# koide3/glim

Measured on NVIDIA H100. Metric: VGICP linearize throughput, higher is better.
Workload: dtype f32

## Files before the change

glim_b200/csrc/gb_api.cu:

```cuda
#include "gb_internal.cuh"
#include "gb_grid_math.cuh"

#include <stdarg.h>
#include <stdio.h>
#include <stdlib.h>
#include <string.h>

#include <algorithm>
#include <atomic>
#include <cmath>
#include <map>
#include <mutex>
#include <new>
#include <thread>

static thread_local char g_err[512] = "";
void gb_set_error(const char* fmt, ...) {
  va_list ap;
  va_start(ap, fmt);
  vsnprintf(g_err, sizeof(g_err), fmt, ap);
  va_end(ap);
}
extern "C" const char* gb_last_error(void) { return g_err; }
extern "C" const char* gb_status_string(gb_status s) {
// ... 327 lines not shown
  return GB_OK;
}

static gb_status grid_factor_args(const gb_ctx* ctx, const gb_point_grid* target, const gb_cloud* source, double max_correspondence_distance, bool icp, gb_factor** out,
                                  float* max_corr2, int* half_width) {
  GB_REQUIRE(ctx && target && source && out, "null argument");
  *out = nullptr;
  GB_REQUIRE(std::isfinite(max_correspondence_distance) && max_correspondence_distance > 0.0, "max_correspondence_distance must be positive and finite");
  const gb_voxelmap* m = grid_map(target);
  GB_REQUIRE(m->kind == GB_MAP_POINTS, "the target is not a point grid (gb_point_grid_build)");
  GB_REQUIRE(m->device == ctx->device && source->device == ctx->device, "cloud / point grid live on another device");
  GB_REQUIRE(icp || source->covs, "the source carries no covariances");
  *max_corr2 = (float)(max_correspondence_distance * max_correspondence_distance);
  *half_width = grid_half_width(m->inv_res, *max_corr2, m->key_extent);
  GB_REQUIRE(*half_width <= kGridMaxHalfWidth, "max_correspondence_distance / cell_size too large: the search would span more than 17^3 cells");
  return GB_OK;
}
extern "C" gb_status gb_gicp_grid_factor_create(gb_ctx* ctx, const gb_point_grid* target, const gb_cloud* source, double max_correspondence_distance, gb_factor** out) {
  float max_corr2 = 0.f;
  int half_width = 0;
  GB_CHECK(grid_factor_args(ctx, target, source, max_correspondence_distance, false, out, &max_corr2, &half_width));
  GB_ENTER(ctx);
  gb_factor* f = factor_new(ctx, GB_FACTOR_POSE, grid_map(target), source);
  if (!f) return GB_ERR_INTERNAL;
  f->max_corr2 = max_corr2;
  f->grid_m = half_width;
  *out = f;
  return GB_OK;
}
extern "C" gb_status gb_icp_grid_factor_create(gb_ctx* ctx, const gb_point_grid* target, const gb_cloud* source, double max_correspondence_distance, gb_factor** out) {
  float max_corr2 = 0.f;
  int half_width = 0;
  GB_CHECK(grid_factor_args(ctx, target, source, max_correspondence_distance, true, out, &max_corr2, &half_width));
  GB_ENTER(ctx);
  gb_factor* f = factor_new(ctx, GB_FACTOR_POSE, grid_map(target), source);
  if (!f) return GB_ERR_INTERNAL;
  f->max_corr2 = max_corr2;
  f->grid_m = half_width;
  f->icp = true;
  *out = f;
  return GB_OK;
}
extern "C" gb_status gb_gicp_grid_factor_half_width(const gb_factor* f, int* m) {
  GB_REQUIRE(f && m, "null argument");
  GB_ENTER(f->ctx);
  *m = f->grid_m;
  return GB_OK;
}

static void pool_put(gb_ctx* ctx, const gb_pool_block& b) {
  if (!b.d || !b.h) { pool_block_free(b); return; }
  if (ctx->pool.size() >= 64) {
    size_t k = 0;
    for (size_t i = 1; i < ctx->pool.size(); i++) if (ctx->pool[i].d_cap < ctx->pool[k].d_cap) k = i;
    pool_block_free(ctx->pool[k]);
    ctx->pool.erase(ctx->pool.begin() + k);
  }
  ctx->pool.push_back(b);
}
static bool pool_get(gb_ctx* ctx, size_t d_need, size_t h_need, gb_pool_block* out) {
  int best = -1;
  for (size_t i = 0; i < ctx->pool.size(); i++) {
    const gb_pool_block& b = ctx->pool[i];
    if (b.d_cap >= d_need && b.h_cap >= h_need && b.d_cap <= 4 * d_need + (1 << 16) && (best < 0 || b.d_cap < ctx->pool[best].d_cap)) best = (int)i;
  }
  if (best < 0) return false;
  *out = ctx->pool[best];
  ctx->pool.erase(ctx->pool.begin() + best);
  return true;
}

void sweep_free(gb_sweep* s) {
  if (!s) return;
  gb_ctx* ctx = s->ctx;
  {
    GB_LOCK(ctx);
    cudaSetDevice(ctx->device);
    cudaStreamSynchronize(ctx->stream);
    {
      std::lock_guard<std::mutex> reg(g_registry_mu);
      for (gb_factor* f : s->factors) {
        if (!f) continue;
        auto it = std::find(f->users.begin(), f->users.end(), s);
        if (it != f->users.end()) f->users.erase(it);
      }
    }
    for (int k = 0; k < 2; k++) if (s->pose_ev[k]) cudaEventDestroy(s->pose_ev[k]);
    if (s->graph_exec) cudaGraphExecDestroy(s->graph_exec);
    if (s->d_pair_ptr) cudaFree(s->d_pair_ptr);
    pool_put(ctx, s->blk);
    delete s;
  }
  ctx_release(ctx);
}

extern "C" gb_status gb_vgicp_factor_destroy(gb_factor* f) {
  if (!f) return GB_OK;
  if (f->single) { sweep_free(f->single); f->single = nullptr; }
  {
    std::lock_guard<std::mutex> reg(g_registry_mu);
    for (gb_sweep* s : f->users) {
      s->stale = true;
      for (auto& p : s->factors) if (p == f) p = nullptr;
    }
    f->users.clear();
  }
  gb_ctx* ctx = f->ctx;
  delete f;
  ctx_release(ctx);
  return GB_OK;
}

static int env_int(const char* name, int dflt) {
  const char* v = getenv(name);
  return v && *v ? atoi(v) : dflt;
}

static void build_items(gb_sweep* s, FactorDesc* descs, std::vector<int2>& tiles) {
  tiles.clear();
  const size_t F = s->F;
  if (s->kernel_version == 3) {
    constexpr double kTaperQuarter = 1.5, kTaperSixteenth = 0.4;
    const double warps = (double)s->capacity * 8.0;
    uint64_t total = 0;
    for (size_t f = 0; f < F; f++) total += (uint64_t)descs[f].n;
    const uint64_t tail16 = (uint64_t)(warps * s->tile_size * kTaperSixteenth);
    const uint64_t tail4 = (uint64_t)(warps * s->tile_size * kTaperQuarter);
    uint64_t before = 0;
    for (size_t f = 0; f < F; f++) {
      FactorDesc& D = descs[f];
      const uint64_t remaining = total - before;
      int chunk = s->tile_size;
      if (remaining <= tail16) chunk = std::max(128, s->tile_size / 16);
      else if (remaining <= tail4) chunk = std::max(128, s->tile_size / 4);
      if (total <= (uint64_t)(warps * s->tile_size * 3.0)) chunk = s->tile_size;
      D.chunk = chunk;
      const int nt = std::max(1, (D.n + chunk - 1) / chunk);
      D.num_tiles = nt;
      for (int t = 0; t < nt; t++) tiles.push_back(make_int2((int)f, t * chunk));
      before += (uint64_t)D.n;
    }
    return;
  }
  const double warps = (double)s->capacity * 8.0;
  constexpr int kMinRows = 4;
  std::vector<double> cost(F);
  double tot = 0.0;
  for (size_t f = 0; f < F; f++) {
    const gb_factor* fa = s->factors[f];
    const double r = (fa && fa->inlier_frac >= 0.f) ? (double)fa->inlier_frac : 0.5;
    cost[f] = (double)descs[f].n * (1.0 + 1.25 * r) + 64.0;
    tot += cost[f];
  }
  std::vector<int> J(F);
  double budget = warps;
  for (int iter = 0; iter < 64; iter++) {
    long long sum = 0;
    for (size_t f = 0; f < F; f++) {
      const int rows = (descs[f].n + 31) / 32;
      const int jmax = std::max(1, rows / kMinRows);
      J[f] = std::min(jmax, std::max(1, (int)(cost[f] / tot * budget + 0.5)));
      sum += J[f];
    }
    if ((double)sum <= warps) break;
    budget *= 0.95;
  }
  for (size_t f = 0; f < F; f++) {
    descs[f].chunk = 0;
    descs[f].num_tiles = J[f];
    for (int j = 0; j < J[f]; j++) tiles.push_back(make_int2((int)f, j));
  }
}

static gb_status sweep_learn_inliers(gb_sweep* s) {
  for (size_t f = 0; f < s->F; f++) {
    gb_factor* fa = s->factors[f];
    if (fa && fa->source->n) fa->inlier_frac = (float)(s->h_out[f * GB_OUT_DOUBLES + 121] / (double)fa->source->n);
  }
  if (s->kernel_version != 5 || s->calibrated || s->stale) return GB_OK;
  s->calibrated = true;
  std::vector<int> old(s->F);
  for (size_t f = 0; f < s->F; f++) old[f] = s->h_descs[f].num_tiles;
  std::vector<int2> tiles;
  build_items(s, s->h_descs, tiles);
  bool changed = false;
  for (size_t f = 0; f < s->F; f++) changed = changed || std::abs(old[f] - s->h_descs[f].num_tiles) * 8 > old[f];
  if (!changed || tiles.size() > s->tiles_cap) {
    for (size_t f = 0; f < s->F; f++) s->h_descs[f].num_tiles = old[f];
    return GB_OK;
  }
  memcpy(s->h_tiles, tiles.data(), sizeof(int2) * tiles.size());
  GB_CUDA(cudaMemcpyAsync(s->d_descs, s->h_descs, sizeof(FactorDesc) * s->F, cudaMemcpyHostToDevice, s->ctx->stream));
  GB_CUDA(cudaMemcpyAsync(s->d_tiles, s->h_tiles, sizeof(int2) * tiles.size(), cudaMemcpyHostToDevice, s->ctx->stream));
  s->num_tiles = (int)tiles.size();
  s->grid = std::max(1, std::min((s->num_tiles + 7) / 8, s->capacity));
  if (s->graph_exec) { cudaGraphExecDestroy(s->graph_exec); s->graph_exec = nullptr; }
  if (s->graph_state == 1) s->graph_state = 0;
  return GB_OK;
}

static void desc_target(FactorDesc& D, const gb_voxelmap* t) {
  D.buckets = t->buckets; D.voxels = t->voxels;
  D.mask = (uint32_t)t->num_buckets - 1u;
  D.max_scan = t->max_scan;
  D.inv_res = t->inv_res;
}
void desc_target_gicp(FactorDesc& D, GicpDesc& G, const gb_factor* fa) {
  desc_target(D, fa->target);
  G.cells = fa->target->cells;
  G.max_corr2 = fa->max_corr2;
  G.num_offsets = fa->target->kind == GB_MAP_POINTS ? fa->grid_m : fa->target->mode;
}
static uint64_t factor_bytes(const gb_factor* fa) {
  const bool sv = (fa->flags & GB_FACTOR_SURFACE_VALIDATION) != 0;
  const uint64_t V = (uint64_t)fa->target->num_voxels;
  const uint64_t records = gb_target_class(fa->target) != 0 ? (uint64_t)fa->target->num_points : V;
  uint64_t nb_ref = 16384;
  while (nb_ref < V) nb_ref *= 2;
  if (fa->icp) return ((uint64_t)fa->source->n + records + nb_ref) * 16 + 64 + 488;
  return (uint64_t)fa->source->n * (48 + (sv ? 12 : 0)) + records * 48 + nb_ref * 16 + 64 + 488;
}

static gb_status sweep_follow_targets(gb_sweep* s) {
  if (!s->any_incremental) return GB_OK;
  bool synced = false;
  for (size_t f = 0; f < s->F; f++) {
    const gb_factor* fa = s->factors[f];
    if (!fa || fa->target->version == s->target_versions[f]) continue;
    if (!synced) {
      GB_CUDA(cudaStreamSynchronize(s->ctx->stream));
      synced = true;
    }
    s->target_versions[f] = fa->target->version;
    if (s->gicp) {
      desc_target_gicp(s->h_descs[f], s->h_gdescs[f], fa);
      GB_CUDA(cudaMemcpyAsync(s->d_gdescs + f, s->h_gdescs + f, sizeof(GicpDesc), cudaMemcpyHostToDevice, s->ctx->stream));
    } else {
      desc_target(s->h_descs[f], fa->target);
    }
    GB_CUDA(cudaMemcpyAsync(s->d_descs + f, s->h_descs + f, sizeof(FactorDesc), cudaMemcpyHostToDevice, s->ctx->stream));
  }
  if (synced) {
    s->algorithmic_bytes = 0;
    for (size_t f = 0; f < s->F; f++) if (s->factors[f]) s->algorithmic_bytes += factor_bytes(s->factors[f]);
  }
  return GB_OK;
}

static size_t sweep_layout(gb_sweep* s, Carver& d, Carver& h) {
  const size_t F = s->F;
  s->d_descs = d.take<FactorDesc>(F);
  s->d_tiles = d.take<int2>(s->tiles_cap);
  s->d_poses = d.take<double>(16 * F);
  s->d_poses_eval = d.take<double>(16 * F);
  const size_t zero_from = d.off;
  s->d_accum = d.take<double>(GB_ACC_STRIDE * F * s->acc_slots);
  s->d_done = d.take<unsigned>(F);
  s->d_tile_ctr = d.take<unsigned long long>(1);
  const size_t zero_bytes = d.off - zero_from;
  s->d_out = d.take<double>(GB_OUT_DOUBLES * F);
  s->h_pose_slot[0] = h.take<double>(16 * F);
  s->h_pose_slot[1] = h.take<double>(16 * F);
  s->h_poses_eval = h.take<double>(16 * F);
  s->h_out = h.take<double>(GB_OUT_DOUBLES * F);
  s->h_descs = h.take<FactorDesc>(F);
  s->h_tiles = h.take<int2>(s->tiles_cap);
  s->d_gdescs = s->gicp ? d.take<GicpDesc>(F) : nullptr;
  s->h_gdescs = s->gicp ? h.take<GicpDesc>(F) : nullptr;
  return zero_bytes;
}

extern "C" gb_status gb_sweep_create(gb_ctx* ctx, size_t F, gb_factor* const* factors, const int32_t* pair_index, gb_sweep** out) {
  GB_REQUIRE(ctx && out, "null argument");
  GB_REQUIRE(F == 0 || factors, "null factor list");
  *out = nullptr;
  uint64_t total_pts = 0;
  for (size_t f = 0; f < F; f++) {
    GB_REQUIRE(factors[f], "null factor");
    GB_REQUIRE(factors[f]->kind == GB_FACTOR_POSE,
               "not a pose factor: a CT factor has two poses (the gb_ct_* entry points), a plane factor one per key (gb_plane_evm_*)");
    GB_REQUIRE(factors[f]->source->device == ctx->device && factors[f]->target->device == ctx->device, "factor lives on another device");
    GB_REQUIRE(gb_factor_class(factors[f]) == gb_factor_class(factors[0]),
               "the factors of one sweep must all be VGICP factors, all GICP factors on iVoxes, all GICP factors on point grids or all ICP factors");
    total_pts += factors[f]->source->n;
  }
  const int factor_class = F > 0 ? gb_factor_class(factors[0]) : 0;
  const bool gicp = factor_class != 0;
  GB_REQUIRE(!gicp || !pair_index, "GICP sweeps take no pair_index (no slab can be attached to them)");
  GB_ENTER(ctx);
  gb_owned<gb_sweep> s(new (std::nothrow) gb_sweep(), sweep_free);
  if (!s) return GB_ERR_INTERNAL;
  ctx_retain(ctx);
  s->ctx = ctx; s->F = F; s->factors.assign(factors, factors + F);
  s->gicp = gicp;
  s->point_grid = factor_class >= 2;
  s->icp = factor_class == 3;

  const int kv = env_int("GB_KERNEL", 0);
  s->capacity = ctx->num_sms * 2;
  const uint64_t warps = (uint64_t)s->capacity * 8;
  const bool small = F > 0 && total_pts <= warps * 2048;
  s->kernel_version = (kv == 3 || kv == 5) ? kv : (small ? 5 : 3);
  if (gicp) s->kernel_version = 5;
  {
    constexpr uint64_t kItemsPerWarp = 6, kMinItem = 128, kMaxItem = 2048;
    const uint64_t want = total_pts / (warps * kItemsPerWarp) + 1;
    const int tile = (int)std::min(kMaxItem, std::max(kMinItem, want));
    s->tile_size = (tile + 31) / 32 * 32;
  }

  std::vector<FactorDesc> descs(F);
  std::vector<GicpDesc> gdescs(gicp ? F : 0);
  std::vector<int2> tiles;
  bool any_sv = false;
  for (size_t f = 0; f < F; f++) {
    const gb_factor* fa = factors[f];
    FactorDesc& D = descs[f];
    D.p0 = fa->source->p0; D.p1 = fa->source->p1; D.p2 = fa->source->p2;
    const bool sv = (fa->flags & GB_FACTOR_SURFACE_VALIDATION) != 0;
    D.normals = sv ? fa->source->normals : nullptr;
    any_sv = any_sv || sv;
    if (gicp) desc_target_gicp(D, gdescs[f], fa); else desc_target(D, fa->target);
    s->target_versions.push_back(fa->target->version);
    s->any_incremental = s->any_incremental || (fa->target->kind != GB_MAP_BUILT && fa->target->kind != GB_MAP_POINTS);
    D.n = (int)fa->source->n;
    D.pair = pair_index ? pair_index[f] : (int)f;
    s->h_pair.push_back(D.pair);
    D.flags = fa->flags;
    D.num_tiles = 1; D.chunk = s->tile_size;
    s->point_factors += (uint64_t)D.n;
    s->algorithmic_bytes += factor_bytes(fa);
  }
  s->any_sv = any_sv;
  build_items(s.get(), descs.data(), tiles);
  s->num_tiles = (int)tiles.size();
  s->grid = std::max(1, std::min((s->num_tiles + 7) / 8, s->capacity));
  s->acc_slots = 1;
  while (F > 0 && s->acc_slots < 16 && (uint64_t)s->num_tiles > (uint64_t)F * 64 * s->acc_slots) s->acc_slots *= 2;

  if (F > 0) {
    s->tiles_cap = std::max<size_t>(tiles.size(), s->kernel_version == 5 ? (size_t)warps + F : 0);
    Carver d, h;
    sweep_layout(s.get(), d, h);
    if (!pool_get(ctx, d.off, h.off, &s->blk)) {
      GB_CUDA(cudaMalloc(&s->blk.d, d.off));
      s->blk.d_cap = d.off;
      GB_CUDA(cudaMallocHost(&s->blk.h, h.off));
      s->blk.h_cap = h.off;
    }
    d = Carver{(char*)s->blk.d};
    h = Carver{(char*)s->blk.h};
    const size_t zero_bytes = sweep_layout(s.get(), d, h);
    memcpy(s->h_descs, descs.data(), sizeof(FactorDesc) * F);
    memcpy(s->h_tiles, tiles.data(), sizeof(int2) * tiles.size());
    cudaStream_t st = ctx->stream;
    GB_CUDA(cudaMemcpyAsync(s->d_descs, s->h_descs, sizeof(FactorDesc) * F, cudaMemcpyHostToDevice, st));
    if (gicp) {
      memcpy(s->h_gdescs, gdescs.data(), sizeof(GicpDesc) * F);
      GB_CUDA(cudaMemcpyAsync(s->d_gdescs, s->h_gdescs, sizeof(GicpDesc) * F, cudaMemcpyHostToDevice, st));
    }
    GB_CUDA(cudaMemcpyAsync(s->d_tiles, s->h_tiles, sizeof(int2) * tiles.size(), cudaMemcpyHostToDevice, st));
    GB_CUDA(cudaMemsetAsync(s->d_accum, 0, zero_bytes, st));
    for (int k = 0; k < 2; k++) GB_CUDA(cudaEventCreateWithFlags(&s->pose_ev[k], cudaEventDisableTiming));
  }
  {
    std::lock_guard<std::mutex> reg(g_registry_mu);
    for (gb_factor* f : s->factors) f->users.push_back(s.get());
  }
  *out = s.release();
  return GB_OK;
}
extern "C" gb_status gb_sweep_destroy(gb_sweep* s) { sweep_free(s); return GB_OK; }

extern "C" gb_status gb_sweep_attach_slab(gb_sweep* s, void* device_slab_f32, size_t num_pairs) {
  GB_REQUIRE(s, "null sweep");
  GB_REQUIRE(!s->gicp || !device_slab_f32, "no slab can be attached to a GICP sweep");
  for (size_t f = 0; f < s->F && device_slab_f32; f++)
    GB_REQUIRE(s->h_pair[f] >= 0 && (size_t)s->h_pair[f] < num_pairs, "pair index out of range for this slab");
  s->d_slab = (float*)device_slab_f32;
  s->num_pairs = num_pairs;
  return GB_OK;
}

extern "C" gb_status gb_sweep_set_poses(gb_sweep* s, const double* T) {
  GB_REQUIRE(s && (s->F == 0 || T), "null argument");
  if (s->F == 0) return GB_OK;
  GB_ENTER(s->ctx);
  const int k = s->pose_slot;
  s->pose_slot ^= 1;
  GB_CUDA(cudaEventSynchronize(s->pose_ev[k]));
  memcpy(s->h_pose_slot[k], T, sizeof(double) * 16 * s->F);
  GB_CUDA(cudaMemcpyAsync(s->d_poses, s->h_pose_slot[k], sizeof(double) * 16 * s->F, cudaMemcpyHostToDevice, s->ctx->stream));
  GB_CUDA(cudaEventRecord(s->pose_ev[k], s->ctx->stream));
  return GB_OK;
}
static gb_status sweep_launch(gb_sweep* s, int mode) {
  if (s->stale) { gb_set_error("a factor of this sweep has been destroyed"); return GB_ERR_INVALID_ARGUMENT; }
  GB_CHECK(sweep_follow_targets(s));
  return gb_launch_sweep(s, mode);
}
static gb_status sweep_error(gb_sweep* s, const double* T_lin, const double* T_eval, double* errors) {
  GB_CHECK(gb_sweep_set_poses(s, T_lin));
  memcpy(s->h_poses_eval, T_eval, sizeof(double) * 16 * s->F);
  GB_CUDA(cudaMemcpyAsync(s->d_poses_eval, s->h_poses_eval, sizeof(double) * 16 * s->F, cudaMemcpyHostToDevice, s->ctx->stream));
  GB_CHECK(sweep_launch(s, GB_MODE_ERROR));
  GB_CUDA(cudaMemcpyAsync(s->h_out, s->d_out, sizeof(double) * GB_OUT_DOUBLES * s->F, cudaMemcpyDeviceToHost, s->ctx->stream));
  GB_CUDA(cudaStreamSynchronize(s->ctx->stream));
  for (size_t f = 0; f < s->F; f++) errors[f] = s->h_out[f * GB_OUT_DOUBLES + 120];
  return GB_OK;
}
extern "C" gb_status gb_sweep_launch(gb_sweep* s) {
  GB_REQUIRE(s, "null sweep");
  GB_ENTER(s->ctx);
  return sweep_launch(s, GB_MODE_LINEARIZE);
}
extern "C" gb_status gb_sweep_fetch(gb_sweep* s, gb_linearized6* out) {
  GB_REQUIRE(s && (s->F == 0 || out), "null argument");
  if (s->F == 0) return GB_OK;
  GB_ENTER(s->ctx);
  static_assert(sizeof(gb_linearized6) == sizeof(double) * GB_OUT_DOUBLES, "gb_linearized6 layout");
  GB_CUDA(cudaMemcpyAsync(s->h_out, s->d_out, sizeof(double) * GB_OUT_DOUBLES * s->F, cudaMemcpyDeviceToHost, s->ctx->stream));
  GB_CUDA(cudaStreamSynchronize(s->ctx->stream));
  memcpy(out, s->h_out, sizeof(double) * GB_OUT_DOUBLES * s->F);
  return sweep_learn_inliers(s);
}
extern "C" gb_status gb_sweep_results_device(gb_sweep* s, void** device_ptr) {
  GB_REQUIRE(s && device_ptr, "null argument");
  *device_ptr = s->d_out;
  return GB_OK;
}
extern "C" gb_status gb_sweep_stats(const gb_sweep* s, uint64_t* point_factors, uint64_t* algorithmic_bytes, uint32_t* num_tiles, uint32_t* grid_size) {
  GB_REQUIRE(s, "null sweep");
  if (point_factors) *point_factors = s->point_factors;
  if (algorithmic_bytes) *algorithmic_bytes = s->algorithmic_bytes;
  if (num_tiles) *num_tiles = (uint32_t)s->num_tiles;
  if (grid_size) *grid_size = (uint32_t)s->grid;
  return GB_OK;
}

static gb_status cached_sweep(gb_ctx* ctx, size_t F, gb_factor* const* factors, gb_sweep** out) {
  uint64_t key = 1469598103934665603ull;
  for (size_t f = 0; f < F; f++) {
    GB_REQUIRE(factors[f], "null factor");
    key = (key ^ factors[f]->id) * 1099511628211ull;
  }
  key ^= (uint64_t)F << 48;
  for (size_t i = 0; i < ctx->sweep_cache.size();) {
    if (ctx->sweep_cache[i]->stale) { sweep_free(ctx->sweep_cache[i]); ctx->sweep_cache.erase(ctx->sweep_cache.begin() + i); } else i++;
  }
  for (gb_sweep* s : ctx->sweep_cache)
    if (s->key == key && s->F == F && std::equal(s->factors.begin(), s->factors.end(), factors)) { *out = s; return GB_OK; }
  gb_sweep* s = nullptr;
  GB_CHECK(gb_sweep_create(ctx, F, factors, nullptr, &s));
  s->key = key;
  if (ctx->sweep_cache.size() >= 64) { sweep_free(ctx->sweep_cache.front()); ctx->sweep_cache.erase(ctx->sweep_cache.begin()); }
  ctx->sweep_cache.push_back(s);
  *out = s;
  return GB_OK;
}

static bool graph_eligible(const gb_sweep* s) {
  return s->graph_state >= 0 && s->kernel_version == 5 && !s->peer && !s->d_slab && (unsigned long long)s->num_tiles <= (unsigned long long)s->grid * 8ull && s->F > 0;
}
static gb_status sweep_linearize(gb_sweep* s, const double* T, gb_linearized6* out) {
  if (!graph_eligible(s)) {
    GB_CHECK(gb_sweep_set_poses(s, T));
    GB_CHECK(sweep_launch(s, GB_MODE_LINEARIZE));
    return gb_sweep_fetch(s, out);
  }
  if (s->stale) { gb_set_error("a factor of this sweep has been destroyed"); return GB_ERR_INVALID_ARGUMENT; }
  gb_ctx* ctx = s->ctx;
  GB_CHECK(sweep_follow_targets(s));
  cudaStream_t st = ctx->stream;
  const size_t pose_bytes = sizeof(double) * 16 * s->F, out_bytes = sizeof(double) * GB_OUT_DOUBLES * s->F;
  if (s->graph_state == 0) {
    GB_CUDA(cudaStreamSynchronize(st));
    cudaGraph_t graph = nullptr;
    bool ok = cudaStreamBeginCapture(st, cudaStreamCaptureModeThreadLocal) == cudaSuccess;
    if (ok) {
      ok = cudaMemcpyAsync(s->d_poses, s->h_pose_slot[0], pose_bytes, cudaMemcpyHostToDevice, st) == cudaSuccess;
      const uint64_t launches = ctx->launches;
      ok = ok && gb_launch_sweep(s, GB_MODE_LINEARIZE) == GB_OK;
      ctx->launches = launches;
      ok = ok && cudaMemcpyAsync(s->h_out, s->d_out, out_bytes, cudaMemcpyDeviceToHost, st) == cudaSuccess;
      ok = (cudaStreamEndCapture(st, &graph) == cudaSuccess) && ok && graph != nullptr;
    }
    if (ok) ok = cudaGraphInstantiate(&s->graph_exec, graph, 0) == cudaSuccess;
    if (graph) cudaGraphDestroy(graph);
    if (!ok) {
      cudaGetLastError();
      s->graph_exec = nullptr;
      s->graph_state = -1;
      return sweep_linearize(s, T, out);
    }
    s->graph_state = 1;
  }
  GB_CUDA(cudaEventSynchronize(s->pose_ev[0]));
  memcpy(s->h_pose_slot[0], T, pose_bytes);
  GB_CUDA(cudaGraphLaunch(s->graph_exec, st));
  ctx->launches++;
  GB_CUDA(cudaStreamSynchronize(st));
  memcpy(out, s->h_out, out_bytes);
  return sweep_learn_inliers(s);
}

extern "C" gb_status gb_sweep_linearize(gb_sweep* s, const double* T, gb_linearized6* out) {
  GB_REQUIRE(s && (s->F == 0 || (T && out)), "null argument");
  if (s->F == 0) return GB_OK;
  GB_ENTER(s->ctx);
  return sweep_linearize(s, T, out);
}

extern "C" gb_status gb_factor_set_linearize(gb_ctx* ctx, size_t F, gb_factor* const* factors, const double* T, gb_linearized6* out) {
  GB_REQUIRE(ctx, "null ctx");
  if (F == 0) return GB_OK;
  GB_REQUIRE(factors && T && out, "null argument");
  GB_ENTER(ctx);
  gb_sweep* s = nullptr;
  GB_CHECK(cached_sweep(ctx, F, factors, &s));
  return sweep_linearize(s, T, out);
}

extern "C" gb_status gb_factor_set_error(gb_ctx* ctx, size_t F, gb_factor* const* factors, const double* T_lin, const double* T_eval, double* errors) {
  GB_REQUIRE(ctx, "null ctx");
  if (F == 0) return GB_OK;
  GB_REQUIRE(factors && T_lin && T_eval && errors, "null argument");
  GB_ENTER(ctx);
  gb_sweep* s = nullptr;
  GB_CHECK(cached_sweep(ctx, F, factors, &s));
  return sweep_error(s, T_lin, T_eval, errors);
}

static gb_status single_sweep(gb_factor* f, gb_sweep** out) {
  if (!f->single) GB_CHECK(gb_sweep_create(f->ctx, 1, &f, nullptr, &f->single));
  *out = f->single;
  return GB_OK;
}
extern "C" gb_status gb_vgicp_linearize(gb_factor* f, const double T[16], gb_linearized6* out) {
  GB_REQUIRE(f && T && out, "null argument");
  GB_ENTER(f->ctx);
  gb_sweep* s = nullptr;
  GB_CHECK(single_sweep(f, &s));
  return sweep_linearize(s, T, out);
}
extern "C" gb_status gb_vgicp_error(gb_factor* f, const double T_lin[16], const double T_eval[16], double* error) {
  GB_REQUIRE(f && T_lin && T_eval && error, "null argument");
  GB_ENTER(f->ctx);
  gb_sweep* s = nullptr;
  GB_CHECK(single_sweep(f, &s));
  return sweep_error(s, T_lin, T_eval, error);
}

extern "C" gb_status gb_hessian_blocks(const gb_linearized6* L, double error_scale, double* G11, double* G12, double* g1, double* G22, double* g2, double* f) {
  GB_REQUIRE(L, "null record");
  if (G11) memcpy(G11, L->H_tt, sizeof(double) * 36);
  if (G12) memcpy(G12, L->H_ts, sizeof(double) * 36);
  if (G22) memcpy(G22, L->H_ss, sizeof(double) * 36);
  for (int k = 0; k < 6; k++) {
    if (g1) g1[k] = -L->b_t[k];
    if (g2) g2[k] = -L->b_s[k];
  }
  if (f) *f = error_scale * L->error;
  return GB_OK;
}
extern "C" gb_status gb_slab_row_hessian_blocks(const float* row, double error_scale, double* G11, double* G12, double* g1, double* G22, double* g2, double* f, double* num_inliers) {
  GB_REQUIRE(row, "null slab row");
  int u = 0;
  for (int i = 0; i < 6; i++)
    for (int j = i; j < 6; j++, u++) {
      if (G11) { G11[j * 6 + i] = row[u]; G11[i * 6 + j] = row[u]; }
      if (G22) { G22[j * 6 + i] = row[57 + u]; G22[i * 6 + j] = row[57 + u]; }
    }
  if (G12) for (int e = 0; e < 36; e++) G12[e] = row[21 + e];
  for (int k = 0; k < 6; k++) {
    if (g1) g1[k] = -(double)row[78 + k];
    if (g2) g2[k] = -(double)row[84 + k];
  }
  if (f) *f = error_scale * (double)row[90];
  if (num_inliers) *num_inliers = (double)row[91];
  return GB_OK;
}

extern "C" gb_status gb_overlap(gb_ctx* ctx, size_t T, const gb_voxelmap* const* targets, const gb_cloud* source, const double* deltas, double* overlap) {
  GB_REQUIRE(ctx && source && overlap, "null argument");
  *overlap = 0.0;
  if (T == 0 || source->n == 0) return GB_OK;
  GB_REQUIRE(targets && deltas, "null targets / deltas");
  for (size_t t = 0; t < T; t++) GB_REQUIRE(!targets[t] || targets[t]->kind != GB_MAP_POINTS, "a point grid is not an occupancy target");
  GB_ENTER(ctx);
  struct Staging { FactorDesc* descs; double* poses; int* count; } h, d;
  auto layout = [&](Carver& cv, Staging& b) {
    b.descs = cv.take<FactorDesc>(T);
    b.poses = cv.take<double>(16 * T);
    b.count = cv.take<int>(1);
  };
  GB_CHECK(gb_carve(ctx, ctx->pinned, [&](Carver& cv) { layout(cv, h); }));
  GB_CHECK(gb_carve(ctx, ctx->scratch, [&](Carver& cv) { layout(cv, d); }));
  for (size_t t = 0; t < T; t++) {
    GB_REQUIRE(targets[t], "null target");
    FactorDesc& D = h.descs[t];
    memset(&D, 0, sizeof(D));
    D.p0 = source->p0; D.p1 = source->p1; D.p2 = source->p2;
    desc_target(D, targets[t]);
    D.n = (int)source->n;
  }
  memcpy(h.poses, deltas, sizeof(double) * 16 * T);
// ... 9 lines not shown
```

glim_b200/csrc/gb_kernels_vgicp.cu:

```cuda
#include "gb_internal.cuh"
#include "gb_vgicp_math.cuh"

#include "gb_sweep_steps.cuh"

namespace {

constexpr int kQueue3 = 304;
struct Sweep3Warp {
  uint2 q[kQueue3];
  float acc[29][32];
};
static_assert(sizeof(Sweep3Warp) * kWarps <= 48 * 1024, "static shared memory");
template <int MODE, bool SV> constexpr int kLookupUnroll3 = SV ? 5 : MODE == GB_MODE_LINEARIZE ? 8 : 7;
template <int MODE, bool SV> constexpr int kRound3 = 32 * kLookupUnroll3<MODE, SV> * ((kQueue3 - 31) / (32 * kLookupUnroll3<MODE, SV>));
static_assert(kRound3<GB_MODE_LINEARIZE, false> > 0 && kRound3<GB_MODE_ERROR, false> > 0 && kRound3<GB_MODE_LINEARIZE, true> > 0,
              "a round's hits and the up to 31 carried from the previous round fit the queue");

template <int MODE, bool PEER, bool SV>
__global__ void __launch_bounds__(kThreads, 2) k_vgicp_sweep3(
  const FactorDesc* __restrict__ descs, const double* __restrict__ poses, const double* __restrict__ poses_eval,
  const int2* __restrict__ items, int num_items,
  unsigned long long* __restrict__ item_ctr, unsigned long long ctr_base,
  double* __restrict__ accum, int acc_slots, unsigned* __restrict__ done, double* __restrict__ out, float* __restrict__ slab, const PeerPush* __restrict__ peer) {
  __shared__ __align__(16) Sweep3Warp s_w[kWarps];
  const int lane = threadIdx.x & 31, warp = threadIdx.x >> 5;
  const unsigned lt_mask = (1u << lane) - 1u;
  uint2* __restrict__ q = s_w[warp].q;
  float (*__restrict__ parked)[32] = s_w[warp].acc;
  auto desc_of = [&](int f) { return descs[f]; };
  constexpr int U = kLookupUnroll3<MODE, SV>, kRound = kRound3<MODE, SV>;

  const int total_warps = gridDim.x * kWarps;
  const bool dynamic = num_items > total_warps;
  int item = blockIdx.x * kWarps + warp;
  if (item >= num_items) return;
  int2 it = __ldg(&items[item]);
  int pend_f = -1, pend_last = 0, pend_tiles = 0;
  auto pend_count = [&] { return pend_tiles; };

  while (true) {
    int next_item = 0x7fffffff;
    if (dynamic && lane == 0) next_item = (int)(atomicAdd(item_ctr, 1ull) - ctr_base) + total_warps;
    const int f = it.x;
    const FactorDesc D = descs[f];
    const PoseF P = pose_from_colmajor(poses + (size_t)f * 16);
    PoseF Pe = P;
    if (MODE == GB_MODE_ERROR) Pe = pose_from_colmajor(poses_eval + (size_t)f * 16);
    const int item_end = min(it.y + D.chunk, D.n);
    bool published = pend_f < 0;
    bool held = false;
    auto unpark = [&](float (&acc)[32]) {
#pragma unroll
      for (int k = 0; k < 32; k++) acc[k] = held && k < 29 && (MODE == GB_MODE_LINEARIZE || k >= 27) ? parked[k][lane] : 0.f;
    };

    int nq = 0;
    for (int wb = it.y; wb < item_end; wb += kRound) {
      const int we = min(wb + kRound, item_end);
      for (int i0 = wb; i0 < we; i0 += 32 * U) {
        Probe p[U];
#pragma unroll
        for (int u = 0; u < U; u++) {
          const float4 a0 = __ldg(&D.p0[min(i0 + u * 32 + lane, we - 1)]);
          probe_issue(D, P, a0.x, a0.y, a0.z, p[u]);
        }
        if (!published) {
          published = true;
          __syncwarp();
          if (lane == 0) pend_last = ticket_last(done, pend_f, pend_count);
        }
        int v[U];
        probe_resolve(D, p, v);
#pragma unroll
        for (int u = 0; u < U; u++) probe_compact(v[u], i0 + u * 32 + lane, we, q, nq, lt_mask);
      }
      __syncwarp();
      const int nacc = we == item_end ? nq : (nq & ~31);
      if (nacc > 0) {
        float acc[32];
        unpark(acc);
        accumulate_queue<MODE, SV>(acc, D, P, Pe, q, nacc, lane);
#pragma unroll
        for (int k = 0; k < 29; k++)
          if (MODE == GB_MODE_LINEARIZE || k >= 27) parked[k][lane] = acc[k];
        held = true;
      }
      __syncwarp();
      nq -= nacc;
      if (nacc > 0 && lane < nq) q[lane] = q[nacc + lane];
      __syncwarp();
    }
    if (!published) {
      __syncwarp();
      if (lane == 0) pend_last = ticket_last(done, pend_f, pend_count);
    }

    float acc[32];
    unpark(acc);
    reduce_item<MODE>(acc, accum, f, acc_slots, item, lane);
    if (pend_f >= 0 && __shfl_sync(0xffffffffu, pend_last, 0)) {
      fence_acquire();
      retire_factor<MODE, PEER>(pend_f, desc_of(pend_f), poses, poses_eval, accum, acc_slots, out, slab, peer, q);
      __syncwarp();
    }
    pend_f = f; pend_tiles = D.num_tiles; pend_last = 0;
    item = __shfl_sync(0xffffffffu, next_item, 0);
    if (item >= num_items) break;
    it = __ldg(&items[item]);
  }
  __syncwarp();
  if (lane == 0) pend_last = ticket_last(done, pend_f, pend_count);
  if (__shfl_sync(0xffffffffu, pend_last, 0)) {
    fence_acquire();
    retire_factor<MODE, PEER>(pend_f, desc_of(pend_f), poses, poses_eval, accum, acc_slots, out, slab, peer, q);
  }
}

constexpr int kSubMax = 512;
constexpr int kLookupUnroll5 = 4;
constexpr int kDescCache = 40;
struct CtaCache {
  FactorDesc desc[kDescCache];
  PoseF pose[kDescCache];
  PoseF pose_eval[kDescCache];
};

template <int MODE, bool PEER>
__global__ void __launch_bounds__(kThreads, 2) k_vgicp_sweep5(
  const FactorDesc* __restrict__ descs, int num_factors, const double* __restrict__ poses, const double* __restrict__ poses_eval,
  const int2* __restrict__ items, int num_items,
  unsigned long long* __restrict__ item_ctr, unsigned long long ctr_base,
  double* __restrict__ accum, int acc_slots, unsigned* __restrict__ done, double* __restrict__ out, float* __restrict__ slab, const PeerPush* __restrict__ peer) {
  __shared__ __align__(16) uint2 s_q[kWarps][kSubMax];
  __shared__ CtaCache cache_s;
  CtaCache* const cache = &cache_s;
  constexpr int U = kLookupUnroll5;
  constexpr int kGroupsPerRound = kSubMax / (32 * U);
  const int lane = threadIdx.x & 31, warp = threadIdx.x >> 5;
  const unsigned lt_mask = (1u << lane) - 1u;
  uint2* __restrict__ q = s_q[warp];

  const bool cached = num_factors <= kDescCache;
  if (cached) {
    for (int f = threadIdx.x; f < num_factors; f += kThreads) {
      cache->desc[f] = descs[f];
      cache->pose[f] = pose_from_colmajor(poses + (size_t)f * 16);
      if (MODE == GB_MODE_ERROR) cache->pose_eval[f] = pose_from_colmajor(poses_eval + (size_t)f * 16);
    }
    __syncthreads();
  }
  auto desc_of = [&](int f) -> FactorDesc { FactorDesc d; if (cached) d = cache->desc[f]; else d = descs[f]; return d; };

  const int total_warps = gridDim.x * kWarps;
  const bool dynamic = num_items > total_warps;
  int item = blockIdx.x * kWarps + warp;
  if (item >= num_items) return;
  int nxt = 0x7fffffff;
  if (dynamic) {
    if (lane == 0) nxt = (int)(atomicAdd(item_ctr, 1ull) - ctr_base) + total_warps;
    nxt = __shfl_sync(0xffffffffu, nxt, 0);
  }
  int2 it = __ldg(&items[item]);
  int pend_f = -1, pend_last = 0;
  auto pend_count = [&] { return desc_of(pend_f).num_tiles; };

  while (true) {
    int nxt2 = 0x7fffffff;
    if (dynamic && lane == 0) nxt2 = (int)(atomicAdd(item_ctr, 1ull) - ctr_base) + total_warps;
    int2 it_next = make_int2(0, 0);
    if (nxt < num_items) it_next = __ldg(&items[nxt]);
    const int f = it.x;
    const FactorDesc D = desc_of(f);
    PoseF P;
    if (cached) P = cache->pose[f]; else P = pose_from_colmajor(poses + (size_t)f * 16);
    PoseF Pe = P;
    if (MODE == GB_MODE_ERROR) { if (cached) Pe = cache->pose_eval[f]; else Pe = pose_from_colmajor(poses_eval + (size_t)f * 16); }

    const int limit = D.n;
    const int row_stride = D.num_tiles * 32;
    const int first = it.y * 32;
    int ngroups = 0;
    if (first < limit) {
      const int rows = (limit - first + row_stride - 1) / row_stride;
      ngroups = (rows + U - 1) / U;
    }

    float acc[32];
#pragma unroll
    for (int k = 0; k < 32; k++) acc[k] = 0.f;
    bool published = (pend_f < 0);

    for (int g0 = 0; g0 < ngroups; g0 += kGroupsPerRound) {
      const int g1 = min(g0 + kGroupsPerRound, ngroups);
      int nq = 0;
      float ax[U], ay[U], az[U];
#pragma unroll
      for (int u = 0; u < U; u++) {
        const int i = first + (g0 * U + u) * row_stride + lane;
        const float4 a0 = __ldg(&D.p0[i < limit ? i : 0]);
        ax[u] = a0.x; ay[u] = a0.y; az[u] = a0.z;
      }
      for (int g = g0; g < g1; g++) {
        Probe p[U];
#pragma unroll
        for (int u = 0; u < U; u++) probe_issue(D, P, ax[u], ay[u], az[u], p[u]);
        if (!published) {
          published = true;
          __syncwarp();
          if (lane == 0) pend_last = ticket_last(done, pend_f, pend_count);
        }
        int v[U];
        probe_resolve(D, p, v);
#pragma unroll
        for (int u = 0; u < U; u++) probe_compact(v[u], first + (g * U + u) * row_stride + lane, limit, q, nq, lt_mask);
        if (g + 1 < g1) {
#pragma unroll
          for (int u = 0; u < U; u++) {
            const int i = first + ((g + 1) * U + u) * row_stride + lane;
            const float4 a0 = __ldg(&D.p0[i < limit ? i : 0]);
            ax[u] = a0.x; ay[u] = a0.y; az[u] = a0.z;
          }
        }
      }
      __syncwarp();
      accumulate_queue<MODE, true>(acc, D, P, Pe, q, nq, lane);
      __syncwarp();
    }
    if (!published) {
      __syncwarp();
      if (lane == 0) pend_last = ticket_last(done, pend_f, pend_count);
    }

    reduce_item<MODE>(acc, accum, f, acc_slots, item, lane);
    if (pend_f >= 0 && __shfl_sync(0xffffffffu, pend_last, 0)) {
      fence_acquire();
      retire_factor<MODE, PEER>(pend_f, desc_of(pend_f), poses, poses_eval, accum, acc_slots, out, slab, peer, q);
      __syncwarp();
    }
    pend_f = f;
    pend_last = 0;
    item = nxt;
    it = it_next;
    nxt = __shfl_sync(0xffffffffu, nxt2, 0);
    if (item >= num_items) break;
  }
  __syncwarp();
  if (lane == 0) pend_last = ticket_last(done, pend_f, pend_count);
  if (__shfl_sync(0xffffffffu, pend_last, 0)) {
    fence_acquire();
    retire_factor<MODE, PEER>(pend_f, desc_of(pend_f), poses, poses_eval, accum, acc_slots, out, slab, peer, q);
  }
}

__global__ void __launch_bounds__(256) k_overlap(int num_targets, const FactorDesc* __restrict__ descs, const double* __restrict__ poses, int n, int* __restrict__ count) {
  extern __shared__ float s_poses[];
  for (int k = threadIdx.x; k < num_targets * 12; k += blockDim.x) {
    const int t = k / 12, e = k % 12;
    const int r = e < 9 ? e / 3 : e - 9, c = e < 9 ? e % 3 : 3;
    s_poses[k] = (float)poses[(size_t)t * 16 + c * 4 + r];
  }
  __syncthreads();
  int local = 0;
  const FactorDesc D0 = descs[0];
  for (int i = blockIdx.x * blockDim.x + threadIdx.x; i < n; i += gridDim.x * blockDim.x) {
    const float4 a0 = __ldg(&D0.p0[i]);
    for (int t = 0; t < num_targets; t++) {
      const PoseF P = load_pose(s_poses + 12 * t);
      float qx, qy, qz;
      transform(P, a0.x, a0.y, a0.z, qx, qy, qz);
      const float sum = (qx + qy) + qz;
      if (!(sum == sum)) continue;
      const float inv_res = descs[t].inv_res;
      const int v = gb_lookup(descs[t].buckets, descs[t].mask, descs[t].max_scan, gb_coord(qx, inv_res), gb_coord(qy, inv_res), gb_coord(qz, inv_res));
      if (v >= 0) { local++; break; }
    }
  }
#pragma unroll
  for (int o = 16; o >= 1; o >>= 1) local += __shfl_xor_sync(0xffffffffu, local, o);
  if ((threadIdx.x & 31) == 0 && local) atomicAdd(count, local);
}

}

template <int MODE, bool PEER>
static gb_status launch5(gb_sweep* s, const double* poses_eval, float* slab, const PeerPush* pp) {
  return gb_launch(s->ctx, "k_vgicp_sweep5", k_vgicp_sweep5<MODE, PEER>, s->grid, kThreads, 0, s->d_descs, (int)s->F, s->d_poses, poses_eval, s->d_tiles, s->num_tiles, s->d_tile_ctr,
                   s->ctr_base, s->d_accum, s->acc_slots, s->d_done, s->d_out, slab, pp);
}

template <int MODE, bool PEER, bool SV>
static gb_status launch3(gb_sweep* s, const double* poses_eval, float* slab, const PeerPush* pp) {
  return gb_launch(s->ctx, "k_vgicp_sweep3", k_vgicp_sweep3<MODE, PEER, SV>, s->grid, kThreads, 0, s->d_descs, s->d_poses, poses_eval, s->d_tiles, s->num_tiles, s->d_tile_ctr,
                   s->ctr_base, s->d_accum, s->acc_slots, s->d_done, s->d_out, slab, pp);
}

gb_status gb_launch_sweep(gb_sweep* s, int mode) {
  if (s->num_tiles == 0) return GB_OK;
  if (s->gicp) return gb_launch_gicp_sweep(s, mode);
  const bool peer = (mode == GB_MODE_LINEARIZE) && s->peer != nullptr;
  const PeerPush* pp = peer ? s->d_peer_tables + s->peer->parity : nullptr;
  float* slab = mode == GB_MODE_LINEARIZE ? s->d_slab : nullptr;
  const double* pe = mode == GB_MODE_ERROR ? s->d_poses_eval : nullptr;
  gb_status st;
  if (s->kernel_version == 3) {
    if (s->any_sv) {
      if (mode == GB_MODE_LINEARIZE) st = peer ? launch3<GB_MODE_LINEARIZE, true, true>(s, pe, slab, pp) : launch3<GB_MODE_LINEARIZE, false, true>(s, pe, slab, pp);
      else st = launch3<GB_MODE_ERROR, false, true>(s, pe, slab, pp);
    } else {
      if (mode == GB_MODE_LINEARIZE) st = peer ? launch3<GB_MODE_LINEARIZE, true, false>(s, pe, slab, pp) : launch3<GB_MODE_LINEARIZE, false, false>(s, pe, slab, pp);
      else st = launch3<GB_MODE_ERROR, false, false>(s, pe, slab, pp);
    }
  } else {
    if (mode == GB_MODE_LINEARIZE) st = peer ? launch5<GB_MODE_LINEARIZE, true>(s, pe, slab, pp) : launch5<GB_MODE_LINEARIZE, false>(s, pe, slab, pp);
    else st = launch5<GB_MODE_ERROR, false>(s, pe, slab, pp);
  }
  GB_CHECK(st);
  const unsigned long long warps = (unsigned long long)s->grid * kWarps;
  if ((unsigned long long)s->num_tiles > warps) s->ctr_base += (s->kernel_version == 3 ? 0ull : warps) + (unsigned long long)s->num_tiles;
  return GB_OK;
}

gb_status gb_launch_overlap(gb_ctx* ctx, int num_targets, const FactorDesc* d_descs, const double* d_poses, int n, int* d_count) {
  if (n <= 0 || num_targets <= 0) return GB_OK;
  const int grid = min((n + 255) / 256, ctx->num_sms * 8);
  return gb_launch(ctx, "k_overlap", k_overlap, grid, 256, (size_t)num_targets * 12 * sizeof(float), num_targets, d_descs, d_poses, n, d_count);
}
```

glim_b200/csrc/gb_sweep_steps.cuh:

```cuda
#pragma once
#include "gb_internal.cuh"
#include "gb_vgicp_math.cuh"

namespace {

static_assert(GB_MODE_LINEARIZE == GB_MODE_LINEARIZE_VALUE, "gb_vgicp_math.cuh mirrors the mode constant");
constexpr int kThreads = 256;
constexpr int kWarps = kThreads / 32;

struct Probe {
  int cx, cy, cz;
  uint32_t h;
  int4 b;
};

__device__ __forceinline__ bool bucket_holds(const int4 b, const Probe& p) { return b.w >= 0 && b.x == p.cx && b.y == p.cy && b.z == p.cz; }

__device__ __forceinline__ void probe_issue(const FactorDesc& D, const PoseF& P, float ax, float ay, float az, Probe& p) {
  float qx, qy, qz;
  transform(P, ax, ay, az, qx, qy, qz);
  p.cx = gb_coord(qx, D.inv_res); p.cy = gb_coord(qy, D.inv_res); p.cz = gb_coord(qz, D.inv_res);
  p.h = gb_hash(p.cx, p.cy, p.cz);
  p.b = __ldg(&D.buckets[p.h & D.mask]);
}

template <int U>
__device__ __forceinline__ void probe_resolve(const FactorDesc& D, Probe (&p)[U], int (&v)[U]) {
  bool next[U];
#pragma unroll
  for (int u = 0; u < U; u++) {
    v[u] = bucket_holds(p[u].b, p[u]) ? p[u].b.w : -1;
    next[u] = p[u].b.w >= 0 && v[u] < 0 && D.max_scan > 1;
  }
#pragma unroll
  for (int u = 0; u < U; u++)
    if (next[u]) p[u].b = __ldg(&D.buckets[(p[u].h + 1u) & D.mask]);
#pragma unroll
  for (int u = 0; u < U; u++) {
    if (next[u] && p[u].b.w >= 0) {
      if (bucket_holds(p[u].b, p[u])) {
        v[u] = p[u].b.w;
      } else {
        for (int k = 2; k < D.max_scan; k++) {
          const int4 bb = __ldg(&D.buckets[(p[u].h + (uint32_t)k) & D.mask]);
          if (bb.w < 0) break;
          if (bucket_holds(bb, p[u])) { v[u] = bb.w; break; }
        }
      }
    }
  }
}

__device__ __forceinline__ void probe_compact(int v, int i, int limit, uint2* __restrict__ q, int& nq, unsigned lt_mask) {
  if (i >= limit) v = -1;
  const unsigned m = __ballot_sync(0xffffffffu, v >= 0);
  if (v >= 0) q[nq + __popc(m & lt_mask)] = make_uint2((unsigned)i, (unsigned)v);
  nq += __popc(m);
}

template <int STEP>
__device__ __forceinline__ void reduce_scatter_stage(float (&v)[32], int lane) {
  const bool upper = (lane & STEP) != 0;
#pragma unroll
  for (int j = 0; j < STEP; j++) {
    const float send = upper ? v[j] : v[j + STEP];
    const float keep = upper ? v[j + STEP] : v[j];
    v[j] = keep + __shfl_xor_sync(0xffffffffu, send, STEP);
  }
}

__device__ __forceinline__ float warp_reduce_scatter32(float (&v)[32], int lane) {
  reduce_scatter_stage<16>(v, lane);
  reduce_scatter_stage<8>(v, lane);
  reduce_scatter_stage<4>(v, lane);
  reduce_scatter_stage<2>(v, lane);
  reduce_scatter_stage<1>(v, lane);
  return v[0];
}

__device__ __forceinline__ unsigned ticket_release(unsigned* p) {
  unsigned r;
  asm volatile("atom.add.release.gpu.global.u32 %0, [%1], 1;" : "=r"(r) : "l"(p) : "memory");
  return r;
}
__device__ __forceinline__ void fence_acquire() { asm volatile("fence.acq_rel.gpu;" ::: "memory"); }

__device__ __noinline__ void pair_push(const FactorDesc& D, const double* __restrict__ out, const PeerPush* __restrict__ peer_tab, float* row ) {
  const PeerPush& peer = *peer_tab;
  const int lane = threadIdx.x & 31;
  __syncwarp();
  int last = 0;
  const int pb = peer.pair_ptr[D.pair], pe = peer.pair_ptr[D.pair + 1];
  if (lane == 0) {
    const unsigned t = ticket_release(&peer.pair_done[D.pair]);
    last = (t == (unsigned)(pe - pb) - 1u);
    if (last) peer.pair_done[D.pair] = 0u;
  }
  last = __shfl_sync(0xffffffffu, last, 0);
  if (!last) return;
  fence_acquire();
  for (int e = lane; e < GB_SLAB_STRIDE; e += 32) {
    double s = 0.0;
    if (e < 92) {
      const int r = slab_to_record(e);
      for (int k = pb; k < pe; k++) s += __ldcg(&out[(size_t)peer.pair_factors[k] * GB_OUT_DOUBLES + r]);
    }
    row[e] = (float)s;
  }
  __syncwarp();
  if (lane < GB_SLAB_STRIDE / 4) {
    const float4 v = reinterpret_cast<const float4*>(row)[lane];
    for (int p = 0; p < peer.world; p++) reinterpret_cast<float4*>(peer.base[p] + (size_t)D.pair * GB_SLAB_STRIDE)[lane] = v;
  }
}

constexpr int kEpilogueDoubles = 104;
constexpr int kPairRowOffset = 2 * kEpilogueDoubles;
__device__ __noinline__ void factor_epilogue(int f, const FactorDesc& D, const double* __restrict__ poses, double* __restrict__ accum, int acc_slots, double* __restrict__ out, float* __restrict__ slab, double* sm) {
  const int lane = threadIdx.x & 31;
  double* A = sm;
  double* Ad = sm + 32;
  double* X = sm + 68;
  if (lane < 29) {
    double a = 0.0;
    for (int sl = 0; sl < acc_slots; sl++) {
      double* slot = &accum[((size_t)f * acc_slots + sl) * GB_ACC_STRIDE + lane];
      a += __ldcg(slot);
      *slot = 0.0;
    }
    A[lane] = a;
  }
  const double* T = poses + (size_t)f * 16;
  for (int e = lane; e < 36; e += 32) {
    const int i = e / 6, j = e % 6;
    double v = 0.0;
    if (j < 3 || i >= 3) {
      const int ri = i % 3, cj = j % 3;
      if ((i < 3) == (j < 3)) {
        v = (double)(float)T[cj * 4 + ri];
      } else {
        const double t0 = (double)(float)T[12], t1 = (double)(float)T[13], t2 = (double)(float)T[14];
        const double r0 = (double)(float)T[cj * 4 + 0], r1 = (double)(float)T[cj * 4 + 1], r2 = (double)(float)T[cj * 4 + 2];
        v = ri == 0 ? t1 * r2 - t2 * r1 : (ri == 1 ? t2 * r0 - t0 * r2 : t0 * r1 - t1 * r0);
      }
    }
    Ad[e] = v;
  }
  __syncwarp();
  auto H = [&](int i, int j) -> double {
    const int a = i < j ? i : j, b = i < j ? j : i;
    return A[a * 6 - (a * (a - 1)) / 2 + (b - a)];
  };
  for (int e = lane; e < 36; e += 32) {
    const int i = e / 6, j = e % 6;
    double s = 0;
    for (int k = 0; k < 6; k++) s += H(i, k) * Ad[k * 6 + j];
    X[e] = s;
  }
  __syncwarp();
  double* o = out + (size_t)f * GB_OUT_DOUBLES;
  float* srow = slab ? slab + (size_t)D.pair * GB_SLAB_STRIDE : nullptr;
  for (int e = lane; e < 36; e += 32) {
    const int i = e / 6, j = e % 6;
    double ss = 0;
    for (int k = 0; k < 6; k++) ss += Ad[k * 6 + i] * X[k * 6 + j];
    const double hij = H(i, j);
    o[j * 6 + i] = hij;
    o[36 + j * 6 + i] = ss;
    o[72 + j * 6 + i] = -X[i * 6 + j];
    if (srow) {
      atomicAdd(&srow[21 + j * 6 + i], (float)(-X[i * 6 + j]));
      if (j >= i) {
        const int u = i * 6 - (i * (i - 1)) / 2 + (j - i);
        atomicAdd(&srow[u], (float)hij);
        atomicAdd(&srow[57 + u], (float)ss);
      }
    }
  }
  if (lane < 6) {
    double bs = 0;
    for (int k = 0; k < 6; k++) bs += Ad[k * 6 + lane] * A[21 + k];
    o[108 + lane] = A[21 + lane];
    o[114 + lane] = -bs;
    if (srow) { atomicAdd(&srow[78 + lane], (float)A[21 + lane]); atomicAdd(&srow[84 + lane], (float)(-bs)); }
  }
  if (lane == 6) { o[120] = A[27]; if (srow) atomicAdd(&srow[90], (float)A[27]); }
  if (lane == 7) { o[121] = A[28]; if (srow) atomicAdd(&srow[91], (float)A[28]); }
  __syncwarp();
}

template <int MODE, bool SV>
__device__ __forceinline__ void accumulate_queue(float (&acc)[32], const FactorDesc& D, const PoseF& P, const PoseF& Pe, const uint2* __restrict__ q, int nq, int lane) {
#pragma unroll 2
  for (int k = lane; k < nq; k += 32) {
    const uint2 e = q[k];
    const int i = (int)e.x;
    const float4 a0 = __ldg(&D.p0[i]);
    const float4 a1 = __ldg(&D.p1[i]);
    const float a2 = __ldg(&D.p2[i]);
    const float4 v0 = __ldg(&D.voxels[3 * (size_t)e.y + 0]);
    const float4 v1 = __ldg(&D.voxels[3 * (size_t)e.y + 1]);
    const float4 v2 = __ldg(&D.voxels[3 * (size_t)e.y + 2]);
    if (!SV || D.normals == nullptr || surface_ok(P, __ldg(&D.normals[i]), v0.w, v1.x, v1.y, v1.z, v1.w, v2.x)) accumulate_hit<MODE>(acc, Pe, a0, a1, a2, v0, v1, v2);
  }
}

template <int MODE>
__device__ __forceinline__ void accumulate_icp_queue(float (&acc)[32], const FactorDesc& D, const PoseF& Pe, const uint2* __restrict__ q, int nq, int lane) {
#pragma unroll 2
  for (int k = lane; k < nq; k += 32) {
    const uint2 e = q[k];
    accumulate_icp_hit<MODE>(acc, Pe, __ldg(&D.p0[e.x]), __ldg(&D.voxels[3 * (size_t)e.y]));
  }
}

template <int MODE>
__device__ __forceinline__ void reduce_item(float (&acc)[32], double* __restrict__ accum, int f, int acc_slots, int item, int lane) {
  double* __restrict__ my_acc = accum + ((size_t)f * acc_slots + (size_t)(item & (acc_slots - 1))) * GB_ACC_STRIDE;
  if (MODE == GB_MODE_LINEARIZE) {
    const float r = warp_reduce_scatter32(acc, lane);
    if (lane < 29) atomicAdd(&my_acc[lane], (double)r);
  } else {
    float e = acc[27], n = acc[28];
#pragma unroll
    for (int o = 16; o >= 1; o >>= 1) { e += __shfl_xor_sync(0xffffffffu, e, o); n += __shfl_xor_sync(0xffffffffu, n, o); }
    if (lane == 27) atomicAdd(&my_acc[27], (double)e);
    if (lane == 28) atomicAdd(&my_acc[28], (double)n);
  }
}

template <class NumTiles>
__device__ __forceinline__ int ticket_last(unsigned* __restrict__ done, int f, const NumTiles& num_tiles) {
  const unsigned t = ticket_release(&done[f]);
  const int last = (t == (unsigned)num_tiles() - 1u);
  if (last) done[f] = 0u;
  return last;
}

template <int MODE, bool PEER>
__device__ __forceinline__ void retire_factor(int f, const FactorDesc& D, const double* __restrict__ poses, const double* __restrict__ poses_eval,
                                              double* __restrict__ accum, int acc_slots, double* __restrict__ out, float* __restrict__ slab, const PeerPush* __restrict__ peer, uint2* q) {
  factor_epilogue(f, D, MODE == GB_MODE_ERROR ? poses_eval : poses, accum, acc_slots, out, slab, reinterpret_cast<double*>(q));
  if (PEER && MODE == GB_MODE_LINEARIZE) pair_push(D, out, peer, reinterpret_cast<float*>(q) + kPairRowOffset);
}

}
```

Baseline: 114,200.

## Pack sweep3 hit queue into 32-bit entries and enlarge queue via dynamic smem

The per-warp hit queue in the sweep3 kernel now stores each hit as one 32-bit word: the point offset relative to the item start sits in the high bits and the voxel index in the low 21 bits. This replaces the uint2 entries. The queue grows to about 1055 entries, which makes each accumulation round longer (except with surface validation). Shared memory becomes dynamic and is opted in through cudaFuncSetAttribute. Larger shared memory per block may reduce occupancy, and factors with unbuilt maps or too many voxels to fit the packing are forced onto kernel 5.

Measured after the change: 118,100 (median of 6 runs). 1.03x the previous value.

```diff
diff --git a/glim_b200/csrc/gb_api.cu b/glim_b200/csrc/gb_api.cu
--- a/glim_b200/csrc/gb_api.cu
+++ b/glim_b200/csrc/gb_api.cu
@@ -653,6 +653,10 @@
   const bool small = F > 0 && total_pts <= warps * 2048;
   s->kernel_version = (kv == 3 || kv == 5) ? kv : (small ? 5 : 3);
   if (gicp) s->kernel_version = 5;
+  for (size_t f = 0; f < F; f++) {
+    const gb_voxelmap* t = factors[f]->target;
+    if (t->kind != GB_MAP_BUILT || t->num_voxels >= (1 << 21)) s->kernel_version = 5;
+  }
   {
     constexpr uint64_t kItemsPerWarp = 6, kMinItem = 128, kMaxItem = 2048;
     const uint64_t want = total_pts / (warps * kItemsPerWarp) + 1;
diff --git a/glim_b200/csrc/gb_kernels_vgicp.cu b/glim_b200/csrc/gb_kernels_vgicp.cu
--- a/glim_b200/csrc/gb_kernels_vgicp.cu
+++ b/glim_b200/csrc/gb_kernels_vgicp.cu
@@ -5,14 +5,14 @@
 
 namespace {
 
-constexpr int kQueue3 = 304;
-struct Sweep3Warp {
-  uint2 q[kQueue3];
+constexpr int kQueue3 = 4 * 256 + 31;
+struct __align__(16) Sweep3Warp {
+  unsigned q[kQueue3];
   float acc[29][32];
 };
-static_assert(sizeof(Sweep3Warp) * kWarps <= 48 * 1024, "static shared memory");
+constexpr size_t kSmem3 = sizeof(Sweep3Warp) * kWarps;
 template <int MODE, bool SV> constexpr int kLookupUnroll3 = SV ? 5 : MODE == GB_MODE_LINEARIZE ? 8 : 7;
-template <int MODE, bool SV> constexpr int kRound3 = 32 * kLookupUnroll3<MODE, SV> * ((kQueue3 - 31) / (32 * kLookupUnroll3<MODE, SV>));
+template <int MODE, bool SV> constexpr int kRound3 = 32 * kLookupUnroll3<MODE, SV> * (SV ? 1 : (kQueue3 - 31) / (32 * kLookupUnroll3<MODE, SV>));
 static_assert(kRound3<GB_MODE_LINEARIZE, false> > 0 && kRound3<GB_MODE_ERROR, false> > 0 && kRound3<GB_MODE_LINEARIZE, true> > 0,
               "a round's hits and the up to 31 carried from the previous round fit the queue");
 
@@ -22,10 +22,11 @@
   const int2* __restrict__ items, int num_items,
   unsigned long long* __restrict__ item_ctr, unsigned long long ctr_base,
   double* __restrict__ accum, int acc_slots, unsigned* __restrict__ done, double* __restrict__ out, float* __restrict__ slab, const PeerPush* __restrict__ peer) {
-  __shared__ __align__(16) Sweep3Warp s_w[kWarps];
+  extern __shared__ __align__(16) unsigned char s_sweep3[];
+  Sweep3Warp* const s_w = reinterpret_cast<Sweep3Warp*>(s_sweep3);
   const int lane = threadIdx.x & 31, warp = threadIdx.x >> 5;
   const unsigned lt_mask = (1u << lane) - 1u;
-  uint2* __restrict__ q = s_w[warp].q;
+  unsigned* __restrict__ q = s_w[warp].q;
   float (*__restrict__ parked)[32] = s_w[warp].acc;
   auto desc_of = [&](int f) { return descs[f]; };
   constexpr int U = kLookupUnroll3<MODE, SV>, kRound = kRound3<MODE, SV>;
@@ -72,14 +73,14 @@
         int v[U];
         probe_resolve(D, p, v);
 #pragma unroll
-        for (int u = 0; u < U; u++) probe_compact(v[u], i0 + u * 32 + lane, we, q, nq, lt_mask);
+        for (int u = 0; u < U; u++) probe_compact(v[u], i0 + u * 32 + lane, we, it.y, q, nq, lt_mask);
       }
       __syncwarp();
       const int nacc = we == item_end ? nq : (nq & ~31);
       if (nacc > 0) {
         float acc[32];
         unpark(acc);
-        accumulate_queue<MODE, SV>(acc, D, P, Pe, q, nacc, lane);
+        accumulate_queue<MODE, SV>(acc, D, P, Pe, q, nacc, lane, it.y);
 #pragma unroll
         for (int k = 0; k < 29; k++)
           if (MODE == GB_MODE_LINEARIZE || k >= 27) parked[k][lane] = acc[k];
@@ -290,7 +291,8 @@
 
 template <int MODE, bool PEER, bool SV>
 static gb_status launch3(gb_sweep* s, const double* poses_eval, float* slab, const PeerPush* pp) {
-  return gb_launch(s->ctx, "k_vgicp_sweep3", k_vgicp_sweep3<MODE, PEER, SV>, s->grid, kThreads, 0, s->d_descs, s->d_poses, poses_eval, s->d_tiles, s->num_tiles, s->d_tile_ctr,
+  GB_CUDA(cudaFuncSetAttribute(k_vgicp_sweep3<MODE, PEER, SV>, cudaFuncAttributeMaxDynamicSharedMemorySize, (int)kSmem3));
+  return gb_launch(s->ctx, "k_vgicp_sweep3", k_vgicp_sweep3<MODE, PEER, SV>, s->grid, kThreads, kSmem3, s->d_descs, s->d_poses, poses_eval, s->d_tiles, s->num_tiles, s->d_tile_ctr,
                    s->ctr_base, s->d_accum, s->acc_slots, s->d_done, s->d_out, slab, pp);
 }
 
diff --git a/glim_b200/csrc/gb_sweep_steps.cuh b/glim_b200/csrc/gb_sweep_steps.cuh
--- a/glim_b200/csrc/gb_sweep_steps.cuh
+++ b/glim_b200/csrc/gb_sweep_steps.cuh
@@ -57,6 +57,19 @@
   if (v >= 0) q[nq + __popc(m & lt_mask)] = make_uint2((unsigned)i, (unsigned)v);
   nq += __popc(m);
 }
+
+constexpr int kQueueVoxelBits = 21;
+constexpr unsigned kQueueVoxelMask = (1u << kQueueVoxelBits) - 1u;
+
+__device__ __forceinline__ void probe_compact(int v, int i, int limit, int base, unsigned* __restrict__ q, int& nq, unsigned lt_mask) {
+  if (i >= limit) v = -1;
+  const unsigned m = __ballot_sync(0xffffffffu, v >= 0);
+  if (v >= 0) q[nq + __popc(m & lt_mask)] = ((unsigned)(i - base) << kQueueVoxelBits) | (unsigned)v;
+  nq += __popc(m);
+}
+
+__device__ __forceinline__ uint2 queue_hit(const uint2 e, int) { return e; }
+__device__ __forceinline__ uint2 queue_hit(const unsigned e, int base) { return make_uint2((unsigned)base + (e >> kQueueVoxelBits), e & kQueueVoxelMask); }
 
 template <int STEP>
 __device__ __forceinline__ void reduce_scatter_stage(float (&v)[32], int lane) {
@@ -189,11 +202,11 @@
   __syncwarp();
 }
 
-template <int MODE, bool SV>
-__device__ __forceinline__ void accumulate_queue(float (&acc)[32], const FactorDesc& D, const PoseF& P, const PoseF& Pe, const uint2* __restrict__ q, int nq, int lane) {
+template <int MODE, bool SV, class QE>
+__device__ __forceinline__ void accumulate_queue(float (&acc)[32], const FactorDesc& D, const PoseF& P, const PoseF& Pe, const QE* __restrict__ q, int nq, int lane, int base = 0) {
 #pragma unroll 2
   for (int k = lane; k < nq; k += 32) {
-    const uint2 e = q[k];
+    const uint2 e = queue_hit(q[k], base);
     const int i = (int)e.x;
     const float4 a0 = __ldg(&D.p0[i]);
     const float4 a1 = __ldg(&D.p1[i]);
@@ -239,9 +252,9 @@
 
 template <int MODE, bool PEER>
 __device__ __forceinline__ void retire_factor(int f, const FactorDesc& D, const double* __restrict__ poses, const double* __restrict__ poses_eval,
-                                              double* __restrict__ accum, int acc_slots, double* __restrict__ out, float* __restrict__ slab, const PeerPush* __restrict__ peer, uint2* q) {
-  factor_epilogue(f, D, MODE == GB_MODE_ERROR ? poses_eval : poses, accum, acc_slots, out, slab, reinterpret_cast<double*>(q));
-  if (PEER && MODE == GB_MODE_LINEARIZE) pair_push(D, out, peer, reinterpret_cast<float*>(q) + kPairRowOffset);
-}
-
-}
+                                              double* __restrict__ accum, int acc_slots, double* __restrict__ out, float* __restrict__ slab, const PeerPush* __restrict__ peer, void* q) {
+  factor_epilogue(f, D, MODE == GB_MODE_ERROR ? poses_eval : poses, accum, acc_slots, out, slab, static_cast<double*>(q));
+  if (PEER && MODE == GB_MODE_LINEARIZE) pair_push(D, out, peer, static_cast<float*>(q) + kPairRowOffset);
+}
+
+}
```
